# chanchanchan97/ICAFusion

Hardware: AMD Instinct MI355X
Metric: RGB/IR image-pairs/sec (two-stream forward + NMS) (higher is better)
Workload: dtype bf16

## Files before the change

icafusion_amd/csrc/dmff_wide.hip:

```cpp
#include <type_traits>
#include "icaf_common.h"
#include "conv_common.h"

namespace icaf {

struct WideP {
    const void* x;
    const void* att;
    float* part;
    const float* x32;
    float* y32;
    void* qkv;
    void* y;
    const void* wqkv; const float* bqkv;
    const void* wo; const float* bo;
    const void* w1; const float* b1;
    const void* w2; const float* b2;
    const float* ln_a_g[2]; const float* ln_a_b[2];
    const float* ln_m_g; const float* ln_m_b;
    long long wqkv_gs, bqkv_gs, wo_gs, bo_gs, w1_gs, b1_gs, w2_gs, b2_gs, x_gs, y_gs;
    long long rows;
    int C, Kp, Kp4, hid, ldy;
    int qkv_npass;
    float eps_a, eps_m;
    float c_res_a[2], c_acc_a[2], c_res_m[2], c_acc_m[2];
};

constexpr int WROWS = 64;
constexpr int WDEPTH = 4;
template <int NW_, int SL_> struct WG {
    static constexpr int NW = NW_, SL = SL_;
    static constexpr int WT = 64 * NW;
    static constexpr int WPASS = 32 * NW;
    template <int DT> static constexpr int kstep() { return 32 / Elem<DT>::BYTES; }
    template <int DT> static constexpr int ksl() { return kstep<DT>() * SL; }
    template <int DT> static constexpr int nsl2() { return WPASS / ksl<DT>(); }
    static constexpr int TPR = WT / WROWS;
};
using WG8 = WG<8, 4>;
using WG4 = WG<4, 2>;

struct WCursor {
    const u32x4* base;
    int left, seg;
};

template <int WSL, class NEXT>
__device__ __forceinline__ void wfetch(u32x4 (&w)[WSL], WCursor& c, const NEXT& next) {
    if (c.left == 0) return;
#pragma unroll
    for (int k = 0; k < WSL; ++k) w[k] = c.base[k * 64];
    c.base += WSL * 64;
    if (--c.left == 0) { ++c.seg; next(c); }
}

template <int DT, int WSL, class NEXT>
__device__ __forceinline__ void wpass(f32x16 (&acc)[2], const unsigned char* A, int SA, int n, u32x4 (&wq)[WDEPTH][WSL], WCursor& c, const NEXT& next) {
    const int lane = threadIdx.x & 63, l31 = lane & 31, hi = lane >> 5;
    const unsigned char* a0 = A + (size_t)l31 * SA + hi * 16;
    const unsigned char* a1 = a0 + (size_t)32 * SA;
    for (int s = 0; s < n; s += WDEPTH) {
#pragma unroll
        for (int u = 0; u < WDEPTH; ++u) {
#pragma unroll
            for (int k = 0; k < WSL; ++k) {
                const int off = ((s + u) * WSL + k) * 32;
                const u32x4 x0 = *(const u32x4*)(a0 + off);
                const u32x4 x1 = *(const u32x4*)(a1 + off);
                mma_step<DT>(acc[0], wq[u][k], x0);
                mma_step<DT>(acc[1], wq[u][k], x1);
            }
            wfetch<WSL>(wq[u], c, next);
            __builtin_amdgcn_sched_barrier(0);
        }
    }
}

template <int DT, int TPR>
__device__ __forceinline__ void wide_tile_layernorm(unsigned char* tile, int S, int C, const float* __restrict__ gam, const float* __restrict__ bet, float eps) {
    using E = Elem<DT>;
    const int tid = threadIdx.x, row = tid / TPR, part = tid % TPR;
    const int nv = C / E::VEC;
    unsigned char* r = tile + (size_t)row * S;
    float s = 0.0f;
    for (int v = part; v < nv; v += TPR) {
        float t[E::VEC];
        unpack16<DT>(*(const u32x4*)(r + v * 16), t);
#pragma unroll
        for (int j = 0; j < E::VEC; ++j) s += t[j];
    }
    s += __shfl_xor(s, 1); s += __shfl_xor(s, 2);
    if constexpr (TPR == 8) s += __shfl_xor(s, 4);
    const float mean = s / (float)C;
    float q = 0.0f;
    for (int v = part; v < nv; v += TPR) {
        float t[E::VEC];
        unpack16<DT>(*(const u32x4*)(r + v * 16), t);
#pragma unroll
        for (int j = 0; j < E::VEC; ++j) { const float d = t[j] - mean; q += d * d; }
    }
    q += __shfl_xor(q, 1); q += __shfl_xor(q, 2);
    if constexpr (TPR == 8) q += __shfl_xor(q, 4);
    const float rstd = 1.0f / sqrtf(q / (float)C + eps);
    for (int v = part; v < nv; v += TPR) {
        float t[E::VEC], o[E::VEC];
        unpack16<DT>(*(const u32x4*)(r + v * 16), t);
#pragma unroll
        for (int j = 0; j < E::VEC; ++j) o[j] = (t[j] - mean) * rstd * gam[v * E::VEC + j] + bet[v * E::VEC + j];
        *(u32x4*)(r + v * 16) = pack16<DT>(o);
    }
}

__device__ __forceinline__ void wide_place(int bid, int& g, int& idx) { g = (bid & 7) >> 2; idx = (bid >> 3) * 4 + (bid & 3); }
template <int KS> __device__ __forceinline__ void wide_place_ks(int bid, int& g, int& ks, int& idx) {
    const int x = bid & 7, per = 4 / KS;
    g = x >> 2;
    ks = (x & 3) / per;
    idx = (bid >> 3) * per + (x & 3) % per;
}

template <int DT, class G = WG8>
__global__ __launch_bounds__(G::WT) void dmff_wide_ln_qkv_kernel(const WideP p) {
    using E = Elem<DT>;
    using T = typename E::type;
    constexpr int VEC = E::VEC, EB = E::BYTES;
    extern __shared__ __attribute__((aligned(16))) unsigned char smem[];
    const int C = p.C, SA = C * EB + 16;
    unsigned char* tile = smem;
    const int tid = threadIdx.x, lane = tid & 63, l31 = lane & 31, hi = lane >> 5;
    const int wn = __builtin_amdgcn_readfirstlane(tid >> 6);
    const int npass = p.qkv_npass;
    const int ngrp = 3 * (C / G::WPASS) / npass;
    const int ntiles = (int)((p.rows + WROWS - 1) / WROWS);
    int g, idx;
    wide_place(blockIdx.x, g, idx);
    if (idx >= ntiles * ngrp) return;
    const int tile_i = idx / ngrp, grp = idx - tile_i * ngrp;
    const long long r0 = (long long)tile_i * WROWS;
    const int ks_row = p.Kp / G::template kstep<DT>(), nsl = C / G::template ksl<DT>();

    const u32x4* wf = (const u32x4*)((const T*)p.wqkv + g * p.wqkv_gs) + lane;
    auto next = [&](WCursor& c) {
        if (c.seg >= npass) { c.left = 0; return; }
        c.base = wf + (long long)((grp * npass + c.seg) * G::NW + wn) * ks_row * 64;
        c.left = nsl;
    };
    WCursor cur; cur.seg = 0; next(cur);
    u32x4 wq[WDEPTH][G::SL];
#pragma unroll
    for (int u = 0; u < WDEPTH; ++u) wfetch<G::SL>(wq[u], cur, next);

    {
        const T* xg = (const T*)p.x + g * p.x_gs;
        const int nv = C / VEC;
        for (int i = tid; i < WROWS * nv; i += G::WT) {
            const int row = i / nv, v = i - row * nv;
            long long r = r0 + row;
            r = r < p.rows ? r : p.rows - 1;
            *(u32x4*)(tile + (size_t)row * SA + v * 16) = *(const u32x4*)(xg + r * C + v * VEC);
        }
    }
    lds_barrier();
    wide_tile_layernorm<DT, G::TPR>(tile, SA, C, p.ln_a_g[g], p.ln_a_b[g], p.eps_a);
    lds_barrier();

    const float* bias = p.bqkv + g * p.bqkv_gs;
    const int nout = 3 * C;
    T* out = (T*)p.qkv + (long long)g * p.rows * nout;
    for (int j = 0; j < npass; ++j) {
        f32x16 acc[2];
#pragma unroll
        for (int t = 0; t < 2; ++t)
#pragma unroll
            for (int r = 0; r < 16; ++r) acc[t][r] = 0.0f;
        wpass<DT, G::SL>(acc, tile, SA, nsl, wq, cur, next);
        const int nb = (grp * npass + j) * G::WPASS + wn * 32;
#pragma unroll
        for (int t = 0; t < 2; ++t) {
            const long long row = r0 + t * 32 + l31;
            if (row < p.rows) {
#pragma unroll
                for (int q = 0; q < 4; ++q) {
                    const int n = nb + 8 * q + 4 * hi;
                    const f32x4 b = *(const f32x4*)(bias + n);
                    *(typename Quad<DT>::type*)(out + row * nout + n) =
                        pack4<DT>(acc[t][4 * q] + b[0], acc[t][4 * q + 1] + b[1], acc[t][4 * q + 2] + b[2], acc[t][4 * q + 3] + b[3]);
                }
            }
        }
    }
}

template <int DT, int NPW, int KS = 1, class G = WG8, bool R32 = false>
__global__ __launch_bounds__(G::WT) void dmff_wide_proj_mlp_kernel(const WideP p) {
    using E = Elem<DT>;
    using T = typename E::type;
    constexpr int VEC = E::VEC, EB = E::BYTES;
    extern __shared__ __attribute__((aligned(16))) unsigned char smem[];
    const int C = p.C, SA = C * EB + 16;
    constexpr int WPASS = G::WPASS, WT = G::WT, NSL2 = G::template nsl2<DT>(), KST = G::template kstep<DT>();
    constexpr int SH = WPASS * EB + 16;
    unsigned char* T0 = smem;
    unsigned char* Hb = T0 + (size_t)WROWS * SA;
    float* red = (float*)(Hb + (size_t)WROWS * SH);
    float* b1s = red + G::NW * 64;

    const int tid = threadIdx.x, lane = tid & 63, l31 = lane & 31, hi = lane >> 5;
    const int wn = __builtin_amdgcn_readfirstlane(tid >> 6);
    const int ntiles = (int)((p.rows + WROWS - 1) / WROWS);
    int g, tile_i, ksl = 0;
    if constexpr (KS == 1) wide_place(blockIdx.x, g, tile_i);
    else wide_place_ks<KS>(blockIdx.x, g, ksl, tile_i);
    if (tile_i >= ntiles) return;
    const long long r0 = (long long)tile_i * WROWS;
    const int ks_row = p.Kp / KST, ks_row4 = p.Kp4 / KST, nsl = C / G::template ksl<DT>(), nchunk = p.hid / WPASS / KS, chunk0 = ksl * nchunk;

    const u32x4* wof = (const u32x4*)((const T*)p.wo + g * p.wo_gs) + lane;
    const u32x4* w1f = (const u32x4*)((const T*)p.w1 + g * p.w1_gs) + lane;
    const u32x4* w2f = (const u32x4*)((const T*)p.w2 + g * p.w2_gs) + lane;
    auto next = [&](WCursor& c) {
        const int s = c.seg;
        if (s < NPW) { c.base = wof + (long long)(s * G::NW + wn) * ks_row * 64; c.left = nsl; return; }
        const int m = s - NPW, chunk = m / (1 + NPW), r = m - chunk * (1 + NPW);
        if (chunk >= nchunk) { c.left = 0; return; }
        if (r == 0) { c.base = w1f + (long long)((chunk0 + chunk) * G::NW + wn) * ks_row * 64; c.left = nsl; }
        else { c.base = w2f + ((long long)((r - 1) * G::NW + wn) * ks_row4 + (chunk0 + chunk) * (WPASS / KST)) * 64; c.left = NSL2; }
    };
    WCursor cur; cur.seg = 0; next(cur);
    u32x4 wq[WDEPTH][G::SL];
#pragma unroll
    for (int u = 0; u < WDEPTH; ++u) wfetch<G::SL>(wq[u], cur, next);

    {
        const T* att = (const T*)p.att + (long long)g * p.rows * C;
        const int nv = C / VEC;
        for (int i = tid; i < WROWS * nv; i += WT) {
            const int row = i / nv, v = i - row * nv;
            long long r = r0 + row;
            r = r < p.rows ? r : p.rows - 1;
            *(u32x4*)(T0 + (size_t)row * SA + v * 16) = *(const u32x4*)(att + r * C + v * VEC);
        }
        const float* b1 = p.b1 + g * p.b1_gs;
        for (int i = tid; i < p.hid / KS; i += WT) b1s[i] = b1[chunk0 * WPASS + i];
    }
    lds_barrier();

    bool rok[2];
    const T* xres[2];
    T* yrow[2];
    const float* x32row[2];
    float* y32row[2];
#pragma unroll
    for (int t = 0; t < 2; ++t) {
        const long long row = r0 + t * 32 + l31;
        rok[t] = row < p.rows;
        const long long grow = rok[t] ? row : p.rows - 1;
        xres[t] = (const T*)p.x + g * p.x_gs + grow * C;
        yrow[t] = (T*)p.y + g * p.y_gs + grow * p.ldy;
        x32row[t] = (R32 && p.x32) ? p.x32 + ((long long)g * p.rows + grow) * C : nullptr;
        y32row[t] = R32 ? p.y32 + ((long long)g * p.rows + grow) * C : nullptr;
    }
    using XQ = typename std::conditional<R32, f32x4, typename Quad<DT>::type>::type;
    auto xq_pack = [](float a, float b, float c, float d) -> XQ {
        if constexpr (R32) return f32x4{a, b, c, d};
        else return pack4<DT>(a, b, c, d);
    };
    auto xq_unpack = [](const XQ& q, float* f) {
        if constexpr (R32) { f[0] = q[0]; f[1] = q[1]; f[2] = q[2]; f[3] = q[3]; }
        else unpack4<DT>(q, f);
    };

    constexpr bool PARK = NPW >= 2 || KS > 1;
    XQ xatt[NPW][2][4];
    {
        const float* bias = p.bo + g * p.bo_gs;
        const float ca = p.c_acc_a[g], cr = p.c_res_a[g];
#pragma unroll
        for (int i = 0; i < NPW; ++i) {
            f32x16 acc[2];
#pragma unroll
            for (int t = 0; t < 2; ++t)
#pragma unroll
                for (int r = 0; r < 16; ++r) acc[t][r] = 0.0f;
            wpass<DT, G::SL>(acc, T0, SA, nsl, wq, cur, next);
#pragma unroll
            for (int t = 0; t < 2; ++t)
#pragma unroll
                for (int q = 0; q < 4; ++q) {
                    const int n = i * WPASS + wn * 32 + 8 * q + 4 * hi;
                    const f32x4 bv = *(const f32x4*)(bias + n);
                    float rv[4], v[4];
                    if (R32 && x32row[t]) { const f32x4 r4 = *(const f32x4*)(x32row[t] + n); rv[0] = r4[0]; rv[1] = r4[1]; rv[2] = r4[2]; rv[3] = r4[3]; }
                    else unpack4<DT>(*(const typename Quad<DT>::type*)(xres[t] + n), rv);
#pragma unroll
                    for (int j = 0; j < 4; ++j) v[j] = __builtin_fmaf(cr, rv[j], (acc[t][4 * q + j] + bv[j]) * ca);
                    xatt[i][t][q] = xq_pack(v[0], v[1], v[2], v[3]);
                }
        }
    }
    {
        float mean[2], rstd[2];
        float sum[2] = {0.0f, 0.0f};
#pragma unroll
        for (int i = 0; i < NPW; ++i)
#pragma unroll
            for (int t = 0; t < 2; ++t)
#pragma unroll
                for (int q = 0; q < 4; ++q) {
                    float v[4];
                    xq_unpack(xatt[i][t][q], v);
                    sum[t] += (v[0] + v[1]) + (v[2] + v[3]);
                }
#pragma unroll
        for (int t = 0; t < 2; ++t) {
            sum[t] += __shfl_xor(sum[t], 32);
            if (hi == 0) red[wn * 64 + t * 32 + l31] = sum[t];
        }
        lds_barrier();
#pragma unroll
        for (int t = 0; t < 2; ++t) {
            float s = 0.0f;
#pragma unroll
            for (int w = 0; w < G::NW; ++w) s += red[w * 64 + t * 32 + l31];
            mean[t] = s / (float)C;
        }
        lds_barrier();
        float sq[2] = {0.0f, 0.0f};
#pragma unroll
        for (int i = 0; i < NPW; ++i)
#pragma unroll
            for (int t = 0; t < 2; ++t)
#pragma unroll
                for (int q = 0; q < 4; ++q) {
                    float v[4];
                    xq_unpack(xatt[i][t][q], v);
#pragma unroll
                    for (int j = 0; j < 4; ++j) { const float d = v[j] - mean[t]; sq[t] += d * d; }
                }
#pragma unroll
        for (int t = 0; t < 2; ++t) {
            sq[t] += __shfl_xor(sq[t], 32);
            if (hi == 0) red[wn * 64 + t * 32 + l31] = sq[t];
        }
        lds_barrier();
#pragma unroll
        for (int t = 0; t < 2; ++t) {
            float s = 0.0f;
#pragma unroll
            for (int w = 0; w < G::NW; ++w) s += red[w * 64 + t * 32 + l31];
            rstd[t] = 1.0f / sqrtf(s / (float)C + p.eps_m);
        }
#pragma unroll
        for (int i = 0; i < NPW; ++i)
#pragma unroll
            for (int q = 0; q < 4; ++q) {
                const int n = i * WPASS + wn * 32 + 8 * q + 4 * hi;
                const f32x4 gv = *(const f32x4*)(p.ln_m_g + n), bv = *(const f32x4*)(p.ln_m_b + n);
#pragma unroll
                for (int t = 0; t < 2; ++t) {
                    float v[4], o[4];
                    xq_unpack(xatt[i][t][q], v);
#pragma unroll
                    for (int j = 0; j < 4; ++j) o[j] = (v[j] - mean[t]) * rstd[t] * gv[j] + bv[j];
                    *(typename Quad<DT>::type*)(T0 + (size_t)(t * 32 + l31) * SA + n * EB) = pack4<DT>(o[0], o[1], o[2], o[3]);
                    if constexpr (PARK) {
                        if (rok[t] && ksl == 0) {
                            if constexpr (R32) *(f32x4*)(y32row[t] + n) = xatt[i][t][q];
                            else *(typename Quad<DT>::type*)(yrow[t] + n) = xatt[i][t][q];
                        }
                    }
                }
            }
        lds_barrier();
    }
    f32x16 acc2[NPW][2];
#pragma unroll
    for (int i = 0; i < NPW; ++i)
#pragma unroll
        for (int t = 0; t < 2; ++t)
#pragma unroll
            for (int r = 0; r < 16; ++r) acc2[i][t][r] = 0.0f;
    for (int chunk = 0; chunk < nchunk; ++chunk) {
        f32x16 acc[2];
#pragma unroll
        for (int t = 0; t < 2; ++t)
#pragma unroll
            for (int r = 0; r < 16; ++r) acc[t][r] = 0.0f;
        wpass<DT, G::SL>(acc, T0, SA, nsl, wq, cur, next);
        lds_barrier();
#pragma unroll
        for (int t = 0; t < 2; ++t)
#pragma unroll
            for (int q = 0; q < 4; ++q) {
                const int nl = wn * 32 + 8 * q + 4 * hi;
                const f32x4 bv = *(const f32x4*)(b1s + chunk * WPASS + nl);
                *(typename Quad<DT>::type*)(Hb + (size_t)(t * 32 + l31) * SH + nl * EB) =
                    pack4<DT>(apply_act<ICAF_ACT_GELU, DT>(acc[t][4 * q] + bv[0]), apply_act<ICAF_ACT_GELU, DT>(acc[t][4 * q + 1] + bv[1]),
                              apply_act<ICAF_ACT_GELU, DT>(acc[t][4 * q + 2] + bv[2]), apply_act<ICAF_ACT_GELU, DT>(acc[t][4 * q + 3] + bv[3]));
            }
        lds_barrier();
#pragma unroll
        for (int i = 0; i < NPW; ++i) wpass<DT, G::SL>(acc2[i], Hb, SH, NSL2, wq, cur, next);
    }
    if constexpr (KS > 1) {
        float* part = p.part + ((long long)(ksl * 2 + g) * p.rows) * C;
#pragma unroll
        for (int i = 0; i < NPW; ++i)
#pragma unroll
            for (int q = 0; q < 4; ++q) {
                const int n = i * WPASS + wn * 32 + 8 * q + 4 * hi;
#pragma unroll
                for (int t = 0; t < 2; ++t)
                    if (rok[t])
                        *(f32x4*)(part + (r0 + t * 32 + l31) * C + n) = f32x4{acc2[i][t][4 * q], acc2[i][t][4 * q + 1], acc2[i][t][4 * q + 2], acc2[i][t][4 * q + 3]};
            }
    } else {
        const float* b2 = p.b2 + g * p.b2_gs;
        const float ca = p.c_acc_m[g], cr = p.c_res_m[g];
#pragma unroll
        for (int i = 0; i < NPW; ++i)
#pragma unroll
            for (int q = 0; q < 4; ++q) {
                const int n = i * WPASS + wn * 32 + 8 * q + 4 * hi;
                const f32x4 bv = *(const f32x4*)(b2 + n);
#pragma unroll
                for (int t = 0; t < 2; ++t) {
                    float rv[4], v[4];
                    if constexpr (PARK && R32) { const f32x4 r4 = *(const f32x4*)(y32row[t] + n); rv[0] = r4[0]; rv[1] = r4[1]; rv[2] = r4[2]; rv[3] = r4[3]; }
                    else if constexpr (PARK) unpack4<DT>(*(const typename Quad<DT>::type*)(yrow[t] + n), rv);
                    else xq_unpack(xatt[i][t][q], rv);
#pragma unroll
                    for (int j = 0; j < 4; ++j) v[j] = __builtin_fmaf(cr, rv[j], (acc2[i][t][4 * q + j] + bv[j]) * ca);
                    if (rok[t]) {
                        *(typename Quad<DT>::type*)(yrow[t] + n) = pack4<DT>(v[0], v[1], v[2], v[3]);
                        if constexpr (R32) *(f32x4*)(y32row[t] + n) = f32x4{v[0], v[1], v[2], v[3]};
                    }
                }
            }
    }
}

template <int DT, int KS, bool R32 = false>
__global__ __launch_bounds__(256) void dmff_wide_reduce_kernel(const WideP p) {
    using T = typename Elem<DT>::type;
    const int C = p.C, nq = C >> 2;
    const long long total = 2 * p.rows * nq;
    for (long long idx = (long long)blockIdx.x * 256 + threadIdx.x; idx < total; idx += (long long)gridDim.x * 256) {
        const int qn = (int)(idx % nq);
        const long long gr = idx / nq;
        const int g = (int)(gr / p.rows);
        const long long row = gr - (long long)g * p.rows;
        const int n = qn * 4;
        f32x4 sum = *(const f32x4*)(p.part + ((long long)g * p.rows + row) * C + n);
#pragma unroll
        for (int k = 1; k < KS; ++k) {
            const f32x4 v = *(const f32x4*)(p.part + ((long long)(k * 2 + g) * p.rows + row) * C + n);
            sum[0] += v[0]; sum[1] += v[1]; sum[2] += v[2]; sum[3] += v[3];
        }
        const f32x4 bv = *(const f32x4*)(p.b2 + g * p.b2_gs + n);
        T* y = (T*)p.y + g * p.y_gs + row * p.ldy + n;
        float* y32 = R32 ? p.y32 + ((long long)g * p.rows + row) * C + n : nullptr;
        float rv[4], v[4];
        if constexpr (R32) { const f32x4 r4 = *(const f32x4*)y32; rv[0] = r4[0]; rv[1] = r4[1]; rv[2] = r4[2]; rv[3] = r4[3]; }
        else unpack4<DT>(*(const typename Quad<DT>::type*)y, rv);
        const float ca = p.c_acc_m[g], cr = p.c_res_m[g];
#pragma unroll
        for (int j = 0; j < 4; ++j) v[j] = __builtin_fmaf(cr, rv[j], (sum[j] + bv[j]) * ca);
        *(typename Quad<DT>::type*)y = pack4<DT>(v[0], v[1], v[2], v[3]);
        if constexpr (R32) *(f32x4*)y32 = f32x4{v[0], v[1], v[2], v[3]};
    }
}

static int wide_fill(const icaf_dmff_args* a, WideP& p, const char* who) {
    if (!a || !a->x) return fail(ICAF_ERR_ARG, "%s: null pointer", who);
    if (a->dtype != ICAF_BF16 && a->dtype != ICAF_F16 && !(a->dtype == ICAF_F32 && a->C == 128))
        return fail(ICAF_ERR_UNSUPPORTED, "%s: 16-bit types (fp32: the C = 128 parity build only; dtype %d, C = %d)", who, a->dtype, a->C);
    if (a->B < 1 || a->N < 1) return fail(ICAF_ERR_ARG, "%s: bad B/N", who);
    if (a->C != 128 && a->C != 256 && a->C != 512) return fail(ICAF_ERR_UNSUPPORTED, "%s: C=%d (built for 128 [four wavefronts, 128-channel passes] and 256 / 512 [eight, 256-channel passes])", who, a->C);
    if (a->Kp < a->C || a->Kp % (a->dtype == ICAF_F32 ? 32 : 64)) return fail(ICAF_ERR_ARG, "%s: Kp=%d", who, a->Kp);
    p.x = a->x; p.qkv = a->qkv; p.y = a->y; p.att = nullptr; p.part = nullptr;
    p.x32 = a->x32; p.y32 = a->y32;
    if (a->x32 && !a->y32) return fail(ICAF_ERR_ARG, "%s: x32 without y32 (the fp32 residual stream is read AND written by every iteration but the first)", who);
    if (a->y32 && a->dtype == ICAF_F32) return fail(ICAF_ERR_ARG, "%s: the fp32 residual stream belongs to the 16-bit builds", who);
    if ((a->x32 && ((uintptr_t)a->x32 & 15)) || (a->y32 && ((uintptr_t)a->y32 & 15))) return fail(ICAF_ERR_ARG, "%s: x32 / y32 must be 16-byte aligned", who);
    p.wqkv = a->wqkv; p.bqkv = a->bqkv; p.wo = a->wo; p.bo = a->bo; p.w1 = a->w1; p.b1 = a->b1; p.w2 = a->w2; p.b2 = a->b2;
    p.ln_a_g[0] = a->ln_attn_gamma[0]; p.ln_a_g[1] = a->ln_attn_gamma[1]; p.ln_a_b[0] = a->ln_attn_beta[0]; p.ln_a_b[1] = a->ln_attn_beta[1];
    p.ln_m_g = a->ln_mlp_gamma; p.ln_m_b = a->ln_mlp_beta;
    p.wqkv_gs = a->wqkv_gs; p.bqkv_gs = a->bqkv_gs; p.wo_gs = a->wo_gs; p.bo_gs = a->bo_gs; p.w1_gs = a->w1_gs; p.b1_gs = a->b1_gs;
    p.w2_gs = a->w2_gs; p.b2_gs = a->b2_gs; p.x_gs = a->x_gs; p.y_gs = a->y_gs;
    p.rows = (long long)a->B * a->N; p.C = a->C; p.Kp = a->Kp; p.Kp4 = a->Kp4; p.hid = a->hidden; p.ldy = a->ldy;
    p.qkv_npass = a->reserved == 1 ? 1 : 3;
    p.eps_a = a->eps_attn; p.eps_m = a->eps_mlp;
    for (int g = 0; g < 2; ++g) {
        p.c_res_a[g] = a->coef_res_attn[g]; p.c_acc_a[g] = a->coef_acc_attn[g];
        p.c_res_m[g] = a->coef_res_mlp[g]; p.c_acc_m[g] = a->coef_acc_mlp[g];
    }
    return ICAF_OK;
}

template <int DT, class G>
static int launch_wide_ln_qkv(const WideP& p, hipStream_t s) {
    const size_t lds = (size_t)WROWS * (p.C * Elem<DT>::BYTES + 16);
    ICAF_LDS_OPTIN((dmff_wide_ln_qkv_kernel<DT, G>), lds);
    const long long work = ((p.rows + WROWS - 1) / WROWS) * (3 * (p.C / G::WPASS) / p.qkv_npass);
    hipLaunchKernelGGL((dmff_wide_ln_qkv_kernel<DT, G>), dim3((unsigned)(8 * ((work + 3) / 4))), dim3(G::WT), lds, s, p);
    ICAF_LAUNCH_CHECK();
    return ICAF_OK;
}

template <class G>
static size_t wide_proj_mlp_lds(int C, int hid, int eb = 2) {
    return (size_t)WROWS * (C * eb + 16) + (size_t)WROWS * (G::WPASS * eb + 16) + G::NW * 64 * sizeof(float) + (size_t)hid * sizeof(float);
}

template <int DT, int NPW, class G, bool R32 = false>
static int launch_wide_proj_mlp(const WideP& p, hipStream_t s) {
    const size_t lds = wide_proj_mlp_lds<G>(p.C, p.hid, Elem<DT>::BYTES);
    ICAF_LDS_OPTIN((dmff_wide_proj_mlp_kernel<DT, NPW, 1, G, R32>), lds);
    const long long ntiles = (p.rows + WROWS - 1) / WROWS;
    hipLaunchKernelGGL((dmff_wide_proj_mlp_kernel<DT, NPW, 1, G, R32>), dim3((unsigned)(8 * ((ntiles + 3) / 4))), dim3(G::WT), lds, s, p);
    ICAF_LAUNCH_CHECK();
    return ICAF_OK;
}

template <int DT, int NPW, int KS, bool R32 = false>
static int launch_wide_proj_mlp_split(const WideP& p, hipStream_t s) {
    const size_t lds = wide_proj_mlp_lds<WG8>(p.C, p.hid / KS);
    ICAF_LDS_OPTIN((dmff_wide_proj_mlp_kernel<DT, NPW, KS, WG8, R32>), lds);
    const long long ntiles = (p.rows + WROWS - 1) / WROWS, per = 4 / KS;
    hipLaunchKernelGGL((dmff_wide_proj_mlp_kernel<DT, NPW, KS, WG8, R32>), dim3((unsigned)(8 * ((ntiles + per - 1) / per))), dim3(WG8::WT), lds, s, p);
    ICAF_LAUNCH_CHECK();
    return ICAF_OK;
}

template <int DT>
static int dispatch_wide_split(const WideP& p, int ksplit, hipStream_t s) {
    if (p.y32) {
        if (ksplit != 2) return fail(ICAF_ERR_UNSUPPORTED, "icaf_dmff_wide_proj_mlp_split: the fp32 residual stream is built for ksplit = 2");
        return p.C == 256 ? launch_wide_proj_mlp_split<DT, 1, 2, true>(p, s) : launch_wide_proj_mlp_split<DT, 2, 2, true>(p, s);
    }
    if (p.C == 256) return ksplit == 2 ? launch_wide_proj_mlp_split<DT, 1, 2>(p, s) : launch_wide_proj_mlp_split<DT, 1, 4>(p, s);
    return ksplit == 2 ? launch_wide_proj_mlp_split<DT, 2, 2>(p, s) : launch_wide_proj_mlp_split<DT, 2, 4>(p, s);
}

template <int DT>
static int dispatch_wide_ln_qkv(const WideP& p, hipStream_t s) {
    return p.C == 128 ? launch_wide_ln_qkv<DT, WG4>(p, s) : launch_wide_ln_qkv<DT, WG8>(p, s);
}

template <int DT>
static int dispatch_wide_proj_mlp(const WideP& p, hipStream_t s) {
    if (p.y32) {
        if (p.C == 128) return launch_wide_proj_mlp<DT, 1, WG4, true>(p, s);
        if (p.C == 256) return launch_wide_proj_mlp<DT, 1, WG8, true>(p, s);
        return fail(ICAF_ERR_UNSUPPORTED, "icaf_dmff_wide_proj_mlp: the fp32 residual stream at C = 512 is built for the hidden split (ksplit = 2) only");
    }
    if (p.C == 128) return launch_wide_proj_mlp<DT, 1, WG4>(p, s);
    return p.C == 256 ? launch_wide_proj_mlp<DT, 1, WG8>(p, s) : launch_wide_proj_mlp<DT, 2, WG8>(p, s);
}

template <int DT>
static int launch_wide_reduce(const WideP& p, int ksplit, hipStream_t s) {
    const long long items = 2 * p.rows * (p.C / 4);
    long long blocks = (items + 255) / 256;
    if (blocks > 4096) blocks = 4096;
    if (p.y32) {
        if (ksplit != 2) return fail(ICAF_ERR_UNSUPPORTED, "icaf_dmff_wide_reduce: the fp32 residual stream is built for ksplit = 2");
        hipLaunchKernelGGL((dmff_wide_reduce_kernel<DT, 2, true>), dim3((unsigned)blocks), dim3(256), 0, s, p);
    } else if (ksplit == 2) hipLaunchKernelGGL((dmff_wide_reduce_kernel<DT, 2>), dim3((unsigned)blocks), dim3(256), 0, s, p);
    else hipLaunchKernelGGL((dmff_wide_reduce_kernel<DT, 4>), dim3((unsigned)blocks), dim3(256), 0, s, p);
    ICAF_LAUNCH_CHECK();
    return ICAF_OK;
}

}

using namespace icaf;

extern "C" int icaf_dmff_wide_ln_qkv(const icaf_dmff_args* a, icaf_stream_t s) {
    WideP p{};
    int st = wide_fill(a, p, "icaf_dmff_wide_ln_qkv");
    if (st) return st;
    if (!a->qkv || !a->wqkv || !a->bqkv || !a->ln_attn_gamma[0] || !a->ln_attn_gamma[1] || !a->ln_attn_beta[0] || !a->ln_attn_beta[1])
        return fail(ICAF_ERR_ARG, "icaf_dmff_wide_ln_qkv: null pointer");
    if (a->dtype == ICAF_F32) return launch_wide_ln_qkv<ICAF_F32, WG4>(p, S(s));
    return a->dtype == ICAF_BF16 ? dispatch_wide_ln_qkv<ICAF_BF16>(p, S(s)) : dispatch_wide_ln_qkv<ICAF_F16>(p, S(s));
}

extern "C" int icaf_dmff_wide_proj_mlp(const icaf_dmff_args* a, const void* att, icaf_stream_t s) {
    WideP p{};
    int st = wide_fill(a, p, "icaf_dmff_wide_proj_mlp");
    if (st) return st;
    if (!att || !a->y || !a->wo || !a->bo || !a->w1 || !a->b1 || !a->w2 || !a->b2 || !a->ln_mlp_gamma || !a->ln_mlp_beta) return fail(ICAF_ERR_ARG, "icaf_dmff_wide_proj_mlp: null pointer");
    const int wpass = a->C == 128 ? WG4::WPASS : WG8::WPASS;
    if (a->hidden % wpass || a->hidden < wpass || a->Kp4 < a->hidden || a->Kp4 % (a->dtype == ICAF_F32 ? 32 : 64)) return fail(ICAF_ERR_UNSUPPORTED, "icaf_dmff_wide_proj_mlp: hidden width %d must be a multiple of %d", a->hidden, wpass);
    if (a->ldy < a->C || a->ldy % 4) return fail(ICAF_ERR_ARG, "icaf_dmff_wide_proj_mlp: ldy=%d", a->ldy);
    p.att = att;
    if (a->dtype == ICAF_F32) return launch_wide_proj_mlp<ICAF_F32, 1, WG4>(p, S(s));
    return a->dtype == ICAF_BF16 ? dispatch_wide_proj_mlp<ICAF_BF16>(p, S(s)) : dispatch_wide_proj_mlp<ICAF_F16>(p, S(s));
}

extern "C" int icaf_dmff_wide_proj_mlp_split(const icaf_dmff_args* a, const void* att, float* partial, int ksplit, icaf_stream_t s) {
    WideP p{};
    int st = wide_fill(a, p, "icaf_dmff_wide_proj_mlp_split");
    if (st) return st;
    if (!att || !partial || !a->y || !a->wo || !a->bo || !a->w1 || !a->b1 || !a->w2 || !a->b2 || !a->ln_mlp_gamma || !a->ln_mlp_beta) return fail(ICAF_ERR_ARG, "icaf_dmff_wide_proj_mlp_split: null pointer");
    if (ksplit != 2 && ksplit != 4) return fail(ICAF_ERR_ARG, "icaf_dmff_wide_proj_mlp_split: ksplit %d (2 or 4)", ksplit);
    if (a->C == 128 || a->dtype == ICAF_F32) return fail(ICAF_ERR_UNSUPPORTED, "icaf_dmff_wide_proj_mlp_split: C = 128 has no hidden split (its weights are 0.3 MB)");
    if (a->hidden % (WG8::WPASS * ksplit) || a->Kp4 < a->hidden || a->Kp4 % 64) return fail(ICAF_ERR_UNSUPPORTED, "icaf_dmff_wide_proj_mlp_split: hidden width %d must be a multiple of %d", a->hidden, WG8::WPASS * ksplit);
    if (a->ldy < a->C || a->ldy % 4) return fail(ICAF_ERR_ARG, "icaf_dmff_wide_proj_mlp_split: ldy=%d", a->ldy);
    p.att = att;
    p.part = partial;
    return a->dtype == ICAF_BF16 ? dispatch_wide_split<ICAF_BF16>(p, ksplit, S(s)) : dispatch_wide_split<ICAF_F16>(p, ksplit, S(s));
}

extern "C" int icaf_dmff_wide_reduce(const icaf_dmff_args* a, const float* partial, int ksplit, icaf_stream_t s) {
    WideP p{};
    int st = wide_fill(a, p, "icaf_dmff_wide_reduce");
    if (st) return st;
    if (!partial || !a->y || !a->b2) return fail(ICAF_ERR_ARG, "icaf_dmff_wide_reduce: null pointer");
    if (ksplit != 2 && ksplit != 4) return fail(ICAF_ERR_ARG, "icaf_dmff_wide_reduce: ksplit %d (2 or 4)", ksplit);
    if (a->dtype == ICAF_F32) return fail(ICAF_ERR_UNSUPPORTED, "icaf_dmff_wide_reduce: 16-bit types only");
    if (a->ldy < a->C || a->ldy % 4) return fail(ICAF_ERR_ARG, "icaf_dmff_wide_reduce: ldy=%d", a->ldy);
    p.part = const_cast<float*>(partial);
    return a->dtype == ICAF_BF16 ? launch_wide_reduce<ICAF_BF16>(p, ksplit, S(s)) : launch_wide_reduce<ICAF_F16>(p, ksplit, S(s));
}
```

Measured before the change: 16460.

## Prefetch tiles and params into registers, stage biases in LDS, branchless weight cursor

Input tile loads in the LN+QKV and proj+MLP kernels now go into registers first and are issued before the weight prefetch, then written to LDS afterward, so global latencies overlap. LayerNorm gammas/betas and biases are staged once into LDS, and residual and b1 loads are issued before each MMA pass to hide their latency. The weight-fetch cursor becomes branchless: past the end it refetches the last fragment instead of skipping, which removes a divergent early return at the cost of redundant loads. The new code requires C to match a compile-time tile-load count and rejects other widths.

```diff
diff --git a/icafusion_amd/csrc/dmff_wide.hip b/icafusion_amd/csrc/dmff_wide.hip
--- a/icafusion_amd/csrc/dmff_wide.hip
+++ b/icafusion_amd/csrc/dmff_wide.hip
@@ -1,6 +1,7 @@
 #include <type_traits>
 #include "icaf_common.h"
 #include "conv_common.h"
+#include "wide_cursor.h"
 
 namespace icaf {
 
@@ -40,26 +41,21 @@
 using WG8 = WG<8, 4>;
 using WG4 = WG<4, 2>;
 
-struct WCursor {
-    const u32x4* base;
-    int left, seg;
-};
-
-template <int WSL, class NEXT>
-__device__ __forceinline__ void wfetch(u32x4 (&w)[WSL], WCursor& c, const NEXT& next) {
-    if (c.left == 0) return;
-#pragma unroll
-    for (int k = 0; k < WSL; ++k) w[k] = c.base[k * 64];
-    c.base += WSL * 64;
-    if (--c.left == 0) { ++c.seg; next(c); }
-}
-
-template <int DT, int WSL, class NEXT>
-__device__ __forceinline__ void wpass(f32x16 (&acc)[2], const unsigned char* A, int SA, int n, u32x4 (&wq)[WDEPTH][WSL], WCursor& c, const NEXT& next) {
+template <int WSL, class SEGS, class MATS>
+__device__ __forceinline__ void wfetch(u32x4 (&w)[WSL], WCursor& c, const SEGS& segs, const MATS& mats) {
+    const u32x4* b = mats(c.mat) + c.frag * 64 + (threadIdx.x & 63);
+#pragma unroll
+    for (int k = 0; k < WSL; ++k) w[k] = b[k * 64];
+    wcursor_advance(c, WSL, segs);
+}
+
+template <int DT, int WSL, class SEGS, class MATS>
+__device__ __forceinline__ void wpass(f32x16 (&acc)[2], const unsigned char* A, int SA, int n, u32x4 (&wq)[WDEPTH][WSL], WCursor& c, const SEGS& segs, const MATS& mats) {
     const int lane = threadIdx.x & 63, l31 = lane & 31, hi = lane >> 5;
     const unsigned char* a0 = A + (size_t)l31 * SA + hi * 16;
     const unsigned char* a1 = a0 + (size_t)32 * SA;
-    for (int s = 0; s < n; s += WDEPTH) {
+    int s = 0;
+    do {
 #pragma unroll
         for (int u = 0; u < WDEPTH; ++u) {
 #pragma unroll
@@ -70,14 +66,15 @@
                 mma_step<DT>(acc[0], wq[u][k], x0);
                 mma_step<DT>(acc[1], wq[u][k], x1);
             }
-            wfetch<WSL>(wq[u], c, next);
+            wfetch<WSL>(wq[u], c, segs, mats);
             __builtin_amdgcn_sched_barrier(0);
         }
-    }
+        s += WDEPTH;
+    } while (s < n);
 }
 
 template <int DT, int TPR>
-__device__ __forceinline__ void wide_tile_layernorm(unsigned char* tile, int S, int C, const float* __restrict__ gam, const float* __restrict__ bet, float eps) {
+__device__ __forceinline__ void wide_tile_layernorm(unsigned char* tile, int S, int C, const float* gam, const float* bet, float eps) {
     using E = Elem<DT>;
     const int tid = threadIdx.x, row = tid / TPR, part = tid % TPR;
     const int nv = C / E::VEC;
@@ -119,7 +116,7 @@
     idx = (bid >> 3) * per + (x & 3) % per;
 }
 
-template <int DT, class G = WG8>
+template <int DT, class G = WG8, int NT = 4>
 __global__ __launch_bounds__(G::WT) void dmff_wide_ln_qkv_kernel(const WideP p) {
     using E = Elem<DT>;
     using T = typename E::type;
@@ -127,6 +124,8 @@
     extern __shared__ __attribute__((aligned(16))) unsigned char smem[];
     const int C = p.C, SA = C * EB + 16;
     unsigned char* tile = smem;
+    float* lnp = (float*)(tile + (size_t)WROWS * SA);
+    float* bs = lnp + 2 * C;
     const int tid = threadIdx.x, lane = tid & 63, l31 = lane & 31, hi = lane >> 5;
     const int wn = __builtin_amdgcn_readfirstlane(tid >> 6);
     const int npass = p.qkv_npass;
@@ -139,32 +138,43 @@
     const long long r0 = (long long)tile_i * WROWS;
     const int ks_row = p.Kp / G::template kstep<DT>(), nsl = C / G::template ksl<DT>();
 
-    const u32x4* wf = (const u32x4*)((const T*)p.wqkv + g * p.wqkv_gs) + lane;
-    auto next = [&](WCursor& c) {
-        if (c.seg >= npass) { c.left = 0; return; }
-        c.base = wf + (long long)((grp * npass + c.seg) * G::NW + wn) * ks_row * 64;
-        c.left = nsl;
-    };
-    WCursor cur; cur.seg = 0; next(cur);
-    u32x4 wq[WDEPTH][G::SL];
-#pragma unroll
-    for (int u = 0; u < WDEPTH; ++u) wfetch<G::SL>(wq[u], cur, next);
-
+    u32x4 tl[NT];
+    const int nv = C / VEC;
     {
         const T* xg = (const T*)p.x + g * p.x_gs;
-        const int nv = C / VEC;
-        for (int i = tid; i < WROWS * nv; i += G::WT) {
-            const int row = i / nv, v = i - row * nv;
+#pragma unroll
+        for (int it = 0; it < NT; ++it) {
+            const int i = tid + it * G::WT, row = i / nv, v = i - row * nv;
             long long r = r0 + row;
             r = r < p.rows ? r : p.rows - 1;
-            *(u32x4*)(tile + (size_t)row * SA + v * 16) = *(const u32x4*)(xg + r * C + v * VEC);
-        }
-    }
+            tl[it] = *(const u32x4*)(xg + r * C + v * VEC);
+        }
+    }
+    const int nlq = C / 2, nbq = npass * (G::WPASS / 4);
+    const int lqi = tid < nlq ? tid : nlq - 1, bqi = tid < nbq ? tid : nbq - 1;
+    const f32x4 lq = *(const f32x4*)(lqi < C / 4 ? p.ln_a_g[g] + 4 * lqi : p.ln_a_b[g] + 4 * lqi - C);
+    const f32x4 bq = *(const f32x4*)(p.bqkv + g * p.bqkv_gs + grp * npass * G::WPASS + 4 * bqi);
+
+    const u32x4* wf = (const u32x4*)((const T*)p.wqkv + g * p.wqkv_gs);
+    const WQkvSegs segs{npass, grp, G::NW, wn, ks_row, nsl};
+    auto mats = [&](int) { return wf; };
+    WCursor cur;
+    wcursor_start(cur, G::SL, segs);
+    u32x4 wq[WDEPTH][G::SL];
+#pragma unroll
+    for (int u = 0; u < WDEPTH; ++u) wfetch<G::SL>(wq[u], cur, segs, mats);
+
+#pragma unroll
+    for (int it = 0; it < NT; ++it) {
+        const int i = tid + it * G::WT, row = i / nv, v = i - row * nv;
+        *(u32x4*)(tile + (size_t)row * SA + v * 16) = tl[it];
+    }
+    if (tid < nlq) *(f32x4*)(lnp + 4 * tid) = lq;
+    if (tid < nbq) *(f32x4*)(bs + 4 * tid) = bq;
     lds_barrier();
-    wide_tile_layernorm<DT, G::TPR>(tile, SA, C, p.ln_a_g[g], p.ln_a_b[g], p.eps_a);
+    wide_tile_layernorm<DT, G::TPR>(tile, SA, C, lnp, lnp + C, p.eps_a);
     lds_barrier();
 
-    const float* bias = p.bqkv + g * p.bqkv_gs;
     const int nout = 3 * C;
     T* out = (T*)p.qkv + (long long)g * p.rows * nout;
     for (int j = 0; j < npass; ++j) {
@@ -173,19 +183,18 @@
         for (int t = 0; t < 2; ++t)
 #pragma unroll
             for (int r = 0; r < 16; ++r) acc[t][r] = 0.0f;
-        wpass<DT, G::SL>(acc, tile, SA, nsl, wq, cur, next);
+        wpass<DT, G::SL>(acc, tile, SA, nsl, wq, cur, segs, mats);
         const int nb = (grp * npass + j) * G::WPASS + wn * 32;
 #pragma unroll
-        for (int t = 0; t < 2; ++t) {
-            const long long row = r0 + t * 32 + l31;
-            if (row < p.rows) {
-#pragma unroll
-                for (int q = 0; q < 4; ++q) {
-                    const int n = nb + 8 * q + 4 * hi;
-                    const f32x4 b = *(const f32x4*)(bias + n);
+        for (int q = 0; q < 4; ++q) {
+            const int n = nb + 8 * q + 4 * hi;
+            const f32x4 b = *(const f32x4*)(bs + j * G::WPASS + wn * 32 + 8 * q + 4 * hi);
+#pragma unroll
+            for (int t = 0; t < 2; ++t) {
+                const long long row = r0 + t * 32 + l31;
+                if (row < p.rows)
                     *(typename Quad<DT>::type*)(out + row * nout + n) =
                         pack4<DT>(acc[t][4 * q] + b[0], acc[t][4 * q + 1] + b[1], acc[t][4 * q + 2] + b[2], acc[t][4 * q + 3] + b[3]);
-                }
             }
         }
     }
@@ -203,7 +212,8 @@
     unsigned char* T0 = smem;
     unsigned char* Hb = T0 + (size_t)WROWS * SA;
     float* red = (float*)(Hb + (size_t)WROWS * SH);
-    float* b1s = red + G::NW * 64;
+    float* prm = red + G::NW * 64;
+    constexpr int NT = WROWS * (NPW * WPASS / VEC) / WT;
 
     const int tid = threadIdx.x, lane = tid & 63, l31 = lane & 31, hi = lane >> 5;
     const int wn = __builtin_amdgcn_readfirstlane(tid >> 6);
@@ -215,34 +225,38 @@
     const long long r0 = (long long)tile_i * WROWS;
     const int ks_row = p.Kp / KST, ks_row4 = p.Kp4 / KST, nsl = C / G::template ksl<DT>(), nchunk = p.hid / WPASS / KS, chunk0 = ksl * nchunk;
 
-    const u32x4* wof = (const u32x4*)((const T*)p.wo + g * p.wo_gs) + lane;
-    const u32x4* w1f = (const u32x4*)((const T*)p.w1 + g * p.w1_gs) + lane;
-    const u32x4* w2f = (const u32x4*)((const T*)p.w2 + g * p.w2_gs) + lane;
-    auto next = [&](WCursor& c) {
-        const int s = c.seg;
-        if (s < NPW) { c.base = wof + (long long)(s * G::NW + wn) * ks_row * 64; c.left = nsl; return; }
-        const int m = s - NPW, chunk = m / (1 + NPW), r = m - chunk * (1 + NPW);
-        if (chunk >= nchunk) { c.left = 0; return; }
-        if (r == 0) { c.base = w1f + (long long)((chunk0 + chunk) * G::NW + wn) * ks_row * 64; c.left = nsl; }
-        else { c.base = w2f + ((long long)((r - 1) * G::NW + wn) * ks_row4 + (chunk0 + chunk) * (WPASS / KST)) * 64; c.left = NSL2; }
-    };
-    WCursor cur; cur.seg = 0; next(cur);
-    u32x4 wq[WDEPTH][G::SL];
-#pragma unroll
-    for (int u = 0; u < WDEPTH; ++u) wfetch<G::SL>(wq[u], cur, next);
-
+    u32x4 tl[NT];
+    constexpr int NV = NPW * WPASS / VEC;
     {
         const T* att = (const T*)p.att + (long long)g * p.rows * C;
-        const int nv = C / VEC;
-        for (int i = tid; i < WROWS * nv; i += WT) {
-            const int row = i / nv, v = i - row * nv;
+#pragma unroll
+        for (int it = 0; it < NT; ++it) {
+            const int i = tid + it * WT, row = i / NV, v = i - row * NV;
             long long r = r0 + row;
             r = r < p.rows ? r : p.rows - 1;
-            *(u32x4*)(T0 + (size_t)row * SA + v * 16) = *(const u32x4*)(att + r * C + v * VEC);
-        }
-        const float* b1 = p.b1 + g * p.b1_gs;
-        for (int i = tid; i < p.hid / KS; i += WT) b1s[i] = b1[chunk0 * WPASS + i];
-    }
+            tl[it] = *(const u32x4*)(att + r * C + v * VEC);
+        }
+    }
+    const int pqi = tid < C ? tid : C - 1, pw = pqi / (C / 4), po = 4 * pqi - pw * C;
+    const f32x4 pq = *(const f32x4*)((pw == 0 ? p.ln_m_g : pw == 1 ? p.ln_m_b : pw == 2 ? p.bo + g * p.bo_gs : p.b2 + g * p.b2_gs) + po);
+
+    const u32x4* wof = (const u32x4*)((const T*)p.wo + g * p.wo_gs);
+    const u32x4* w1f = (const u32x4*)((const T*)p.w1 + g * p.w1_gs);
+    const u32x4* w2f = (const u32x4*)((const T*)p.w2 + g * p.w2_gs);
+    const WMlpSegs segs{NPW, G::NW, wn, ks_row, ks_row4, nsl, NSL2, nchunk, chunk0, WPASS / KST};
+    auto mats = [&](int m) { return m == 0 ? wof : m == 1 ? w1f : w2f; };
+    WCursor cur;
+    wcursor_start(cur, G::SL, segs);
+    u32x4 wq[WDEPTH][G::SL];
+#pragma unroll
+    for (int u = 0; u < WDEPTH; ++u) wfetch<G::SL>(wq[u], cur, segs, mats);
+
+#pragma unroll
+    for (int it = 0; it < NT; ++it) {
+        const int i = tid + it * WT, row = i / NV, v = i - row * NV;
+        *(u32x4*)(T0 + (size_t)row * SA + v * 16) = tl[it];
+    }
+    if (tid < C) *(f32x4*)(prm + 4 * tid) = pq;
     lds_barrier();
 
     bool rok[2];
@@ -257,9 +271,10 @@
         const long long grow = rok[t] ? row : p.rows - 1;
         xres[t] = (const T*)p.x + g * p.x_gs + grow * C;
         yrow[t] = (T*)p.y + g * p.y_gs + grow * p.ldy;
-        x32row[t] = (R32 && p.x32) ? p.x32 + ((long long)g * p.rows + grow) * C : nullptr;
         y32row[t] = R32 ? p.y32 + ((long long)g * p.rows + grow) * C : nullptr;
-    }
+        x32row[t] = R32 ? (p.x32 ? p.x32 + ((long long)g * p.rows + grow) * C : y32row[t]) : nullptr;
+    }
+    const bool has32 = R32 && p.x32 != nullptr;
     using XQ = typename std::conditional<R32, f32x4, typename Quad<DT>::type>::type;
     auto xq_pack = [](float a, float b, float c, float d) -> XQ {
         if constexpr (R32) return f32x4{a, b, c, d};
@@ -273,16 +288,38 @@
     constexpr bool PARK = NPW >= 2 || KS > 1;
     XQ xatt[NPW][2][4];
     {
-        const float* bias = p.bo + g * p.bo_gs;
+        const float* bias = prm + 2 * C;
         const float ca = p.c_acc_a[g], cr = p.c_res_a[g];
 #pragma unroll
         for (int i = 0; i < NPW; ++i) {
+            constexpr bool AHEAD = !(R32 && NPW > 1);
+            typename Quad<DT>::type xr[2][4];
+            f32x4 xr32[R32 ? 2 : 1][R32 ? 4 : 1];
+            auto request = [&]() {
+#pragma unroll
+                for (int t = 0; t < 2; ++t)
+#pragma unroll
+                    for (int q = 0; q < 4; ++q) {
+                        const int n = i * WPASS + wn * 32 + 8 * q + 4 * hi;
+                        xr[t][q] = *(const typename Quad<DT>::type*)(xres[t] + n);
+                        if constexpr (R32) xr32[t][q] = *(const f32x4*)(x32row[t] + n);
+                    }
+            };
+            if constexpr (AHEAD) request();
             f32x16 acc[2];
 #pragma unroll
             for (int t = 0; t < 2; ++t)
 #pragma unroll
                 for (int r = 0; r < 16; ++r) acc[t][r] = 0.0f;
-            wpass<DT, G::SL>(acc, T0, SA, nsl, wq, cur, next);
+            wpass<DT, G::SL>(acc, T0, SA, nsl, wq, cur, segs, mats);
+            if constexpr (!AHEAD) request();
+#pragma unroll
+            for (int t = 0; t < 2; ++t)
+#pragma unroll
+                for (int q = 0; q < 4; ++q) {
+                    asm volatile("" : "+v"(xr[t][q]));
+                    if constexpr (R32) asm volatile("" : "+v"(xr32[t][q]));
+                }
 #pragma unroll
             for (int t = 0; t < 2; ++t)
 #pragma unroll
@@ -290,8 +327,11 @@
                     const int n = i * WPASS + wn * 32 + 8 * q + 4 * hi;
                     const f32x4 bv = *(const f32x4*)(bias + n);
                     float rv[4], v[4];
-                    if (R32 && x32row[t]) { const f32x4 r4 = *(const f32x4*)(x32row[t] + n); rv[0] = r4[0]; rv[1] = r4[1]; rv[2] = r4[2]; rv[3] = r4[3]; }
-                    else unpack4<DT>(*(const typename Quad<DT>::type*)(xres[t] + n), rv);
+                    unpack4<DT>(xr[t][q], rv);
+                    if constexpr (R32) {
+#pragma unroll
+                        for (int j = 0; j < 4; ++j) rv[j] = has32 ? xr32[t][q][j] : rv[j];
+                    }
 #pragma unroll
                     for (int j = 0; j < 4; ++j) v[j] = __builtin_fmaf(cr, rv[j], (acc[t][4 * q + j] + bv[j]) * ca);
                     xatt[i][t][q] = xq_pack(v[0], v[1], v[2], v[3]);
@@ -355,7 +395,7 @@
 #pragma unroll
             for (int q = 0; q < 4; ++q) {
                 const int n = i * WPASS + wn * 32 + 8 * q + 4 * hi;
-                const f32x4 gv = *(const f32x4*)(p.ln_m_g + n), bv = *(const f32x4*)(p.ln_m_b + n);
+                const f32x4 gv = *(const f32x4*)(prm + n), bv = *(const f32x4*)(prm + C + n);
 #pragma unroll
                 for (int t = 0; t < 2; ++t) {
                     float v[4], o[4];
@@ -380,27 +420,33 @@
         for (int t = 0; t < 2; ++t)
 #pragma unroll
             for (int r = 0; r < 16; ++r) acc2[i][t][r] = 0.0f;
+    const float* b1 = p.b1 + g * p.b1_gs + (long long)chunk0 * WPASS + wn * 32 + 4 * hi;
     for (int chunk = 0; chunk < nchunk; ++chunk) {
+        f32x4 b1q[4];
+#pragma unroll
+        for (int q = 0; q < 4; ++q) b1q[q] = *(const f32x4*)(b1 + chunk * WPASS + 8 * q);
         f32x16 acc[2];
 #pragma unroll
         for (int t = 0; t < 2; ++t)
 #pragma unroll
             for (int r = 0; r < 16; ++r) acc[t][r] = 0.0f;
-        wpass<DT, G::SL>(acc, T0, SA, nsl, wq, cur, next);
+        wpass<DT, G::SL>(acc, T0, SA, nsl, wq, cur, segs, mats);
+#pragma unroll
+        for (int q = 0; q < 4; ++q) asm volatile("" : "+v"(b1q[q]));
         lds_barrier();
 #pragma unroll
         for (int t = 0; t < 2; ++t)
 #pragma unroll
             for (int q = 0; q < 4; ++q) {
                 const int nl = wn * 32 + 8 * q + 4 * hi;
-                const f32x4 bv = *(const f32x4*)(b1s + chunk * WPASS + nl);
+                const f32x4 bv = b1q[q];
                 *(typename Quad<DT>::type*)(Hb + (size_t)(t * 32 + l31) * SH + nl * EB) =
                     pack4<DT>(apply_act<ICAF_ACT_GELU, DT>(acc[t][4 * q] + bv[0]), apply_act<ICAF_ACT_GELU, DT>(acc[t][4 * q + 1] + bv[1]),
                               apply_act<ICAF_ACT_GELU, DT>(acc[t][4 * q + 2] + bv[2]), apply_act<ICAF_ACT_GELU, DT>(acc[t][4 * q + 3] + bv[3]));
             }
         lds_barrier();
 #pragma unroll
-        for (int i = 0; i < NPW; ++i) wpass<DT, G::SL>(acc2[i], Hb, SH, NSL2, wq, cur, next);
+        for (int i = 0; i < NPW; ++i) wpass<DT, G::SL>(acc2[i], Hb, SH, NSL2, wq, cur, segs, mats);
     }
     if constexpr (KS > 1) {
         float* part = p.part + ((long long)(ksl * 2 + g) * p.rows) * C;
@@ -415,7 +461,7 @@
                         *(f32x4*)(part + (r0 + t * 32 + l31) * C + n) = f32x4{acc2[i][t][4 * q], acc2[i][t][4 * q + 1], acc2[i][t][4 * q + 2], acc2[i][t][4 * q + 3]};
             }
     } else {
-        const float* b2 = p.b2 + g * p.b2_gs;
+        const float* b2 = prm + 3 * C;
         const float ca = p.c_acc_m[g], cr = p.c_res_m[g];
 #pragma unroll
         for (int i = 0; i < NPW; ++i)
@@ -498,24 +544,26 @@
     return ICAF_OK;
 }
 
-template <int DT, class G>
+template <int DT, class G, int NT>
 static int launch_wide_ln_qkv(const WideP& p, hipStream_t s) {
-    const size_t lds = (size_t)WROWS * (p.C * Elem<DT>::BYTES + 16);
-    ICAF_LDS_OPTIN((dmff_wide_ln_qkv_kernel<DT, G>), lds);
+    if (WROWS * (p.C / Elem<DT>::VEC) != NT * G::WT) return fail(ICAF_ERR_UNSUPPORTED, "icaf_dmff_wide_ln_qkv: C=%d is not the width this build loads its tile for", p.C);
+    const size_t lds = (size_t)WROWS * (p.C * Elem<DT>::BYTES + 16) + (size_t)(2 * p.C + 3 * G::WPASS) * sizeof(float);
+    ICAF_LDS_OPTIN((dmff_wide_ln_qkv_kernel<DT, G, NT>), lds);
     const long long work = ((p.rows + WROWS - 1) / WROWS) * (3 * (p.C / G::WPASS) / p.qkv_npass);
-    hipLaunchKernelGGL((dmff_wide_ln_qkv_kernel<DT, G>), dim3((unsigned)(8 * ((work + 3) / 4))), dim3(G::WT), lds, s, p);
+    hipLaunchKernelGGL((dmff_wide_ln_qkv_kernel<DT, G, NT>), dim3((unsigned)(8 * ((work + 3) / 4))), dim3(G::WT), lds, s, p);
     ICAF_LAUNCH_CHECK();
     return ICAF_OK;
 }
 
 template <class G>
-static size_t wide_proj_mlp_lds(int C, int hid, int eb = 2) {
-    return (size_t)WROWS * (C * eb + 16) + (size_t)WROWS * (G::WPASS * eb + 16) + G::NW * 64 * sizeof(float) + (size_t)hid * sizeof(float);
+static size_t wide_proj_mlp_lds(int C, int eb = 2) {
+    return (size_t)WROWS * (C * eb + 16) + (size_t)WROWS * (G::WPASS * eb + 16) + G::NW * 64 * sizeof(float) + (size_t)4 * C * sizeof(float);
 }
 
 template <int DT, int NPW, class G, bool R32 = false>
 static int launch_wide_proj_mlp(const WideP& p, hipStream_t s) {
-    const size_t lds = wide_proj_mlp_lds<G>(p.C, p.hid, Elem<DT>::BYTES);
+    if (p.C != NPW * G::WPASS) return fail(ICAF_ERR_UNSUPPORTED, "icaf_dmff_wide_proj_mlp: C=%d is not the width this build loads its tile for", p.C);
+    const size_t lds = wide_proj_mlp_lds<G>(p.C, Elem<DT>::BYTES);
     ICAF_LDS_OPTIN((dmff_wide_proj_mlp_kernel<DT, NPW, 1, G, R32>), lds);
     const long long ntiles = (p.rows + WROWS - 1) / WROWS;
     hipLaunchKernelGGL((dmff_wide_proj_mlp_kernel<DT, NPW, 1, G, R32>), dim3((unsigned)(8 * ((ntiles + 3) / 4))), dim3(G::WT), lds, s, p);
@@ -525,7 +573,8 @@
 
 template <int DT, int NPW, int KS, bool R32 = false>
 static int launch_wide_proj_mlp_split(const WideP& p, hipStream_t s) {
-    const size_t lds = wide_proj_mlp_lds<WG8>(p.C, p.hid / KS);
+    if (p.C != NPW * WG8::WPASS) return fail(ICAF_ERR_UNSUPPORTED, "icaf_dmff_wide_proj_mlp_split: C=%d is not the width this build loads its tile for", p.C);
+    const size_t lds = wide_proj_mlp_lds<WG8>(p.C);
     ICAF_LDS_OPTIN((dmff_wide_proj_mlp_kernel<DT, NPW, KS, WG8, R32>), lds);
     const long long ntiles = (p.rows + WROWS - 1) / WROWS, per = 4 / KS;
     hipLaunchKernelGGL((dmff_wide_proj_mlp_kernel<DT, NPW, KS, WG8, R32>), dim3((unsigned)(8 * ((ntiles + per - 1) / per))), dim3(WG8::WT), lds, s, p);
@@ -545,7 +594,8 @@
 
 template <int DT>
 static int dispatch_wide_ln_qkv(const WideP& p, hipStream_t s) {
-    return p.C == 128 ? launch_wide_ln_qkv<DT, WG4>(p, s) : launch_wide_ln_qkv<DT, WG8>(p, s);
+    if (p.C == 128) return launch_wide_ln_qkv<DT, WG4, 4>(p, s);
+    return p.C == 256 ? launch_wide_ln_qkv<DT, WG8, 4>(p, s) : launch_wide_ln_qkv<DT, WG8, 8>(p, s);
 }
 
 template <int DT>
@@ -583,7 +633,7 @@
     if (st) return st;
     if (!a->qkv || !a->wqkv || !a->bqkv || !a->ln_attn_gamma[0] || !a->ln_attn_gamma[1] || !a->ln_attn_beta[0] || !a->ln_attn_beta[1])
         return fail(ICAF_ERR_ARG, "icaf_dmff_wide_ln_qkv: null pointer");
-    if (a->dtype == ICAF_F32) return launch_wide_ln_qkv<ICAF_F32, WG4>(p, S(s));
+    if (a->dtype == ICAF_F32) return launch_wide_ln_qkv<ICAF_F32, WG4, 8>(p, S(s));
     return a->dtype == ICAF_BF16 ? dispatch_wide_ln_qkv<ICAF_BF16>(p, S(s)) : dispatch_wide_ln_qkv<ICAF_F16>(p, S(s));
 }
 
diff --git a/icafusion_amd/csrc/wide_cursor.h b/icafusion_amd/csrc/wide_cursor.h
--- /dev/null
+++ b/icafusion_amd/csrc/wide_cursor.h
@@ -0,0 +1,61 @@
+#pragma once
+
+#if defined(__HIPCC__) || defined(__CUDACC__)
+#define ICAF_HD __host__ __device__ __forceinline__
+#else
+#define ICAF_HD inline
+#endif
+
+namespace icaf {
+
+struct WSeg {
+    int mat;
+    long long first;
+    int n;
+};
+
+struct WQkvSegs {
+    int npass, grp, NW, wn, ks_row, nsl;
+    ICAF_HD int count() const { return npass; }
+    ICAF_HD WSeg at(int s) const { return WSeg{0, (long long)((grp * npass + s) * NW + wn) * ks_row, nsl}; }
+};
+
+struct WMlpSegs {
+    int NPW, NW, wn, ks_row, ks_row4, nsl, nsl2, nchunk, chunk0, kst_pass;
+    ICAF_HD int count() const { return NPW + nchunk * (1 + NPW); }
+    ICAF_HD WSeg at(int s) const {
+        if (s < NPW) return WSeg{0, (long long)(s * NW + wn) * ks_row, nsl};
+        const int m = s - NPW, chunk = m / (1 + NPW), r = m - chunk * (1 + NPW);
+        if (r == 0) return WSeg{1, (long long)((chunk0 + chunk) * NW + wn) * ks_row, nsl};
+        return WSeg{2, (long long)((r - 1) * NW + wn) * ks_row4 + (long long)(chunk0 + chunk) * kst_pass, nsl2};
+    }
+};
+
+struct WCursor {
+    long long frag;
+    int mat, left, seg;
+};
+
+template <class SEGS>
+ICAF_HD void wcursor_enter(WCursor& c, int WSL, const SEGS& segs) {
+    const int last = segs.count() - 1;
+    const bool end = c.seg > last;
+    const WSeg s = segs.at(end ? last : c.seg);
+    c.mat = s.mat;
+    c.frag = end ? s.first + (long long)(s.n - 1) * WSL : s.first;
+    c.left = end ? 1 : s.n;
+}
+
+template <class SEGS>
+ICAF_HD void wcursor_start(WCursor& c, int WSL, const SEGS& segs) { c.seg = 0; wcursor_enter(c, WSL, segs); }
+
+template <class SEGS>
+ICAF_HD void wcursor_advance(WCursor& c, int WSL, const SEGS& segs) {
+    c.frag += WSL;
+    if (--c.left == 0) {
+        if (c.seg < segs.count()) ++c.seg;
+        wcursor_enter(c, WSL, segs);
+    }
+}
+
+}
```

Measured after the change: 16650, median of 6. +1.2%, better.
